# jepsen-io/comdb2

Hardware: AMD Instinct MI355X
Metric: serializable conflict checks/sec at 1–8 GPUs, % HBM roofline, vs host CPU (higher is better)
Workload: dtype u64

## Files before the change

### comdb2_amd/csrc/hsc_narrow.hip

```cpp
#include "hsc_device.h"
#include "hsc_internal.h"
#include "hsc_reldiff.h"

#include <hip/hip_runtime.h>

#include <algorithm>
#include <type_traits>

namespace hsc {

constexpr uint64_t kKeyPad = ~0ull;

__device__ __forceinline__ bool cnarrow_bound(const NarrowView &nv, uint64_t xg, const uint64_t *xw,
                                              size_t xs, bool upper, uint64_t &code)
{
    uint64_t acc = 0;
    int pos = 0, np = -1, xb = 0;
    for (int l = 0; l <= nv.W; ++l) {
        const uint64_t *cm = nv.cmeta + 8 * l;
        const uint64_t m = cm[0], pt = cm[1];
        uint64_t x = l ? xw[(size_t)(l - 1) * xs] : xg;
        if (np < 0) {
            const uint64_t d = (x ^ pt) & ~m;
            if (d) {
// ... 1240 lines not shown
        if (first[mid] < x)
            lo = mid + 1;
        else
            hi = mid;
    }
    put(lo);
}

static_assert(kTradMaxTiles <= 0xFFFF, "the packed table holds tile counts as u16");

hipError_t narrow_trad_build(const uint64_t *first, uint32_t ntiles, uint32_t m, uint32_t *trad,
                             uint16_t *trad16, hipStream_t s, int logmode)
{
    if (logmode && m < 64) return hipErrorInvalidValue;
    if (ntiles > kTradMaxTiles) return hipErrorInvalidValue;
    k_trad<<<(m + 8 + 255) / 256, 256, 0, s>>>(first, ntiles, m, logmode, trad, trad16);
    return hipGetLastError();
}

struct LocLds {
    uint32_t first, cdir, hist, trad, sbuf, rbuf, bytes;
};
__host__ __device__ inline LocLds loc_lds(const NarrowTiles &nt, uint32_t ntiles)
{
    LocLds L{};
    uint32_t o = 0;
    L.first = o;
    o += 8 * (nt.trad ? ((ntiles + 1) & ~1u) : dir16_lds_entries(nt.tdir));
    L.cdir = o;
    o += nt.rank_lsn32 ? 0 : 8 * dir16_lds_entries(nt.cdir);
    L.hist = o;
    o += 4 * ((ntiles + 3) & ~3u);
    o = (o + 15) & ~15u;
    L.trad = o;
    o += nt.trad ? (uint32_t)narrow_trad16_bytes(nt.trad_m) : 0;
    L.sbuf = o;
    o += nt.rank_lsn32 ? 0 : 8 * kLocTThreads;
    L.rbuf = o;
    o += 4 * (nt.rank_lsn32 ? kLocTThreads / 64 : kLocTThreads);
    L.bytes = o;
    return L;
}

template <int K, int kMode = -1>
__device__ __forceinline__ void trad_count(const uint64_t *first, const uint16_t *T, uint32_t m,
                                           int shift, uint32_t ntiles, const uint64_t (&x)[K],
                                           const bool (&act)[K], uint32_t (&out)[K])
{
    uint32_t l[K], h[K];
    const bool lg = kMode < 0 ? (shift & kTradLog) != 0 : kMode == 1;
    const int sv = shift & 0xFFFF;
#pragma unroll
    for (int k = 0; k < K; ++k) {
        const uint64_t b = lg ? trad_log_bucket(x[k], sv) : x[k] >> sv;
        const bool in = b < m;
        const uint32_t bi = in ? (uint32_t)b : 0;
        l[k] = in ? T[bi] : ntiles;
        h[k] = in ? T[bi + 1] : ntiles;
    }
    for (;;) {
        bool more = false;
#pragma unroll
        for (int k = 0; k < K; ++k) {
            if (l[k] < h[k]) {
                const uint32_t mid = (l[k] + h[k]) >> 1;
                const bool below = first[mid] < x[k];
                l[k] = below ? mid + 1 : l[k];
                h[k] = below ? h[k] : mid;
                more = true;
            }
        }
        if (!more) break;
    }
#pragma unroll
    for (int k = 0; k < K; ++k) out[k] = act[k] ? l[k] : 0;
}

template <int K>
struct LocDefer {
    uint32_t x[K], y[K], q[K];
    uint64_t snap[K];
};

__device__ __forceinline__ void zero_verdicts(const ProbeWork &work, uint32_t g)
{
    uint8_t *v = work.vout;
    const size_t nb = work.n_txn;
    const size_t head = std::min<size_t>(nb, (16 - ((uintptr_t)v & 15)) & 15);
    const size_t pieces = (nb - head) / 16, tail = head + 16 * pieces;
    const size_t t = (size_t)g * kLocTThreads + threadIdx.x, stride = (size_t)work.G * kLocTThreads;
    for (size_t i = t; i < pieces; i += stride) ((u32x4 *)(v + head))[i] = u32x4{0, 0, 0, 0};
    if (t < head) v[t] = 0;
    if (t < nb - tail) v[tail + t] = 0;
    if (work.bitmap)
        for (size_t i = t; i < ((size_t)work.n_txn + 63) / 64; i += stride) work.bitmap[i] = 0;
}

constexpr int kLocGeneral = 0, kLocFastLin = 1, kLocFastLog = 2;
template <int W, bool kTrad, int kShape = kLocGeneral>
__global__ __launch_bounds__(kLocTThreads) void k_locate_t(NarrowView nv, WinView wt, ProbeView p,
                                                           ProbeWork work, NarrowTiles nt,
                                                           uint8_t *verdict)
{
    constexpr bool kFast = kShape != kLocGeneral;
    static_assert(!kFast || (kTrad && (W == 1 || W == 2)), "fast shapes: bucket table, 1 or 2 words");
    constexpr int WR = 2 > W ? 2 : W;
    constexpr int K = 1, S = kLocTP;
    extern __shared__ __attribute__((aligned(16))) uint64_t lds64[];
    const uint32_t ntiles = wt.ntiles;
    const LocLds L = loc_lds(nt, ntiles);
    char *lb = (char *)lds64;
    uint64_t *tfirst = (uint64_t *)(lb + L.first);
    uint64_t *cdir = (uint64_t *)(lb + L.cdir);
    uint32_t *hist = (uint32_t *)(lb + L.hist);
    uint16_t *T = (uint16_t *)(lb + L.trad);
    const int lane = threadIdx.x & 63;
    uint64_t *sb = (uint64_t *)(lb + L.sbuf) + (threadIdx.x & ~63u);
    uint32_t *rb = (uint32_t *)(lb + L.rbuf) + (threadIdx.x & ~63u);
    const uint32_t g = xcd_chunk(blockIdx.x, (work.G + 7) / 8);
    if (g >= work.G) return;
    HSC_STAMP(work, 0, 0);
    if (g == 0 && threadIdx.x < 3) work.item_off[threadIdx.x] = 0;
    const uint32_t c0 = g * work.chunk;
    const uint32_t c1 = min(p.n, c0 + work.chunk);
    uint32_t qq[2][K], gg[2][K], tx[2][K];
    bool valid[2][K];
    uint64_t snap[2][K], xl[2][K][WR], xh[2][K][WR];
    uint4 R0[S][K], R1[S][K];
    uint32_t RT[S][K];
    uint64_t SS[S][K];
    auto load = [&](int s, int buf) {
#pragma unroll
        for (int k = 0; k < K; ++k) {
            const int j = s * K + k;
            qq[buf][k] = c0 + threadIdx.x + kLocTThreads * j;
            valid[buf][k] = qq[buf][k] < c1;
            const uint32_t q = valid[buf][k] ? qq[buf][k] : 0;
            const bool some = kFast || p.n;
            gg[buf][k] = some ? __builtin_nontemporal_load(p.gid + q) : 0;
            snap[buf][k] = some ? __builtin_nontemporal_load(p.snap + q) : 0;
            tx[buf][k] = some ? __builtin_nontemporal_load(p.txn + q) : 0;
#pragma unroll
            for (int w = 0; w < W; ++w) {
                xl[buf][k][w] = some ? __builtin_nontemporal_load(p.lo + (size_t)w * p.n + q) : 0;
                xh[buf][k][w] = some ? __builtin_nontemporal_load(p.hi + (size_t)w * p.n + q) : 0;
            }
        }
    };
    load(0, 0);
    const int tshift = nt.trad_shift;
    u64x2 sf[kTradFirstSlots], st[kTradSlots];
    uint64_t sft = 0;
    u64x2 sd[kDirSlots], sc[kDirSlots];
    if constexpr (kTrad) {
        const u64x2 *src = (const u64x2 *)wt.sp_w;
        const u64x2 *src16 = (const u64x2 *)nt.trad16;
#pragma unroll
        for (int j = 0; j < kTradFirstSlots; ++j) {
            const uint32_t i = threadIdx.x + kLocTThreads * j;
            sf[j] = *(i < ntiles / 2 ? src + i : src16);
        }
        sft = wt.sp_w[ntiles - 1];
#pragma unroll
        for (int j = 0; j < kTradSlots; ++j) {
            const uint32_t i = threadIdx.x + kLocTThreads * j;
            st[j] = src16[i < narrow_trad16_bytes(nt.trad_m) / 16 ? i : 0];
        }
    } else {
        dir16_stage_issue<kLocTThreads>(nt.tdir, sd);
    }
    const bool lsn32 = kFast || nt.rank_lsn32;
    if (!lsn32) dir16_stage_issue<kLocTThreads>(nt.cdir, sc);
    for (uint32_t i = threadIdx.x; i < ntiles; i += kLocTThreads) hist[i] = 0;
    if constexpr (kTrad) {
#pragma unroll
        for (int j = 0; j < kTradFirstSlots; ++j) {
            const uint32_t i = threadIdx.x + kLocTThreads * j;
            if (i < ntiles / 2) ((u64x2 *)tfirst)[i] = sf[j];
        }
        if ((ntiles & 1) && threadIdx.x == 0) tfirst[ntiles - 1] = sft;
#pragma unroll
        for (int j = 0; j < kTradSlots; ++j) {
            const uint32_t i = threadIdx.x + kLocTThreads * j;
            if (i < narrow_trad16_bytes(nt.trad_m) / 16) ((u64x2 *)T)[i] = st[j];
        }
    } else {
        dir16_stage_store<kLocTThreads>(nt.tdir, sd, tfirst);
    }
    if (!lsn32) dir16_stage_store<kLocTThreads>(nt.cdir, sc, cdir);
    __syncthreads();
    HSC_STAMP(work, 0, 1);
    const uint64_t *first = kTrad ? tfirst : wt.sp_w;
    uint64_t fbase[kFast ? W + 1 : 1] = {};
    const int ftz = nv.tz;
    if constexpr (kFast) {
#pragma unroll
        for (int i = 0; i <= W; ++i) fbase[i] = nv.base[i];
    }
    LocDefer<K> dfr;
#pragma unroll
    for (int k = 0; k < K; ++k) dfr.x[k] = 1, dfr.y[k] = 0;
    uint32_t sm[K][4];
    auto commit = [&](int s) {
#pragma unroll
        for (int k = 0; k < K; ++k) {
            uint4 &a = R0[s][k], &b = R1[s][k];
            bool drop_a = false, drop_b = false;
            if constexpr (kFast) {
                const uint32_t qr = a.w >> nt.qshift;
                drop_a = max(sm[k][0], sm[k][1]) < qr;
                drop_b = max(sm[k][2], sm[k][3]) < (b.w >> nt.qshift);
            }
            if (a.x != kNoTile32) {
                if (!drop_a)
                    a.x |= atomicAdd(&hist[a.x >> 12], 0x10001u) & 0xFFFFu;
                else
                    atomicAdd(&hist[a.x >> 12], 0x10000u), a.x = kNoTile32;
            }
            if (b.x != kNoTile32) {
                if (!drop_b)
                    b.x |= atomicAdd(&hist[b.x >> 12], 0x10001u) & 0xFFFFu;
                else
                    atomicAdd(&hist[b.x >> 12], 0x10000u), b.x = kNoTile32;
            }
        }
    };
#pragma unroll
    for (int s = 0; s < S; ++s) {
        const int cb = s & 1;
        uint64_t pm[K], psn[K];
        if (s > 0) {
#pragma unroll
            for (int k = 0; k < K; ++k) {
                pm[k] = dfr.x[k] <= dfr.y[k] ? tiles_max(wt, dfr.x[k], dfr.y[k]) : 0;
                psn[k] = dfr.snap[k];
            }
        }
        if (s + 1 < S) load(s + 1, cb ^ 1);
        uint64_t lo[K], hi[K];
#pragma unroll
        for (int k = 0; k < K; ++k) {
            if constexpr (kFast)
                locate_codes_fast<W>(ftz, fbase, valid[cb][k], gg[cb][k], xl[cb][k], xh[cb][k],
                                     lo[k], hi[k]);
            else
                locate_codes<W>(nv, p, valid[cb][k] ? qq[cb][k] : 0, gg[cb][k], xl[cb][k],
                                xh[cb][k], lo[k], hi[k]);
        }
        uint32_t rs[K];
        if (lsn32) {
#pragma unroll
            for (int k = 0; k < K; ++k) rs[k] = lsn32_rank(snap[cb][k], nt.rank_base);
        } else {
#pragma unroll
            for (int k = 0; k < K; ++k) rs[k] = 0, SS[s][k] = snap[cb][k];
        }
        uint32_t cnt[2 * K];
        {
            uint64_t keys[2 * K];
            bool act[2 * K];
#pragma unroll
            for (int k = 0; k < K; ++k) {
                keys[2 * k] = lo[k];
                keys[2 * k + 1] = dir_le(hi[k]);
                act[2 * k] = act[2 * k + 1] = valid[cb][k] && lo[k] <= hi[k];
            }
            if constexpr (kTrad)
                trad_count<2 * K, kFast ? kShape == kLocFastLog : -1>(tfirst, T, nt.trad_m, tshift,
                                                                      ntiles, keys, act, cnt);
            else
                dir16_count<2 * K>(nt.tdir, tfirst, keys, act, cnt);
        }
        if constexpr (kFast)
            if (s > 0) commit(s - 1);
#pragma unroll
        for (int k = 0; k < K; ++k) {
            dfr.x[k] = 1, dfr.y[k] = 0;
            R0[s][k].x = R1[s][k].x = kNoTile32;
            RT[s][k] = tx[cb][k];
            if constexpr (kFast) sm[k][0] = sm[k][1] = sm[k][2] = sm[k][3] = 0xFFFFFFFFu;
            if (!valid[cb][k]) continue;
            const uint32_t q = qq[cb][k];
            const uint32_t ca = cnt[2 * k], cbt = cnt[2 * k + 1];
            const uint32_t a = ca ? ca - 1 : 0;
            const uint32_t bt = cbt ? cbt - 1 : 0;
            uint4 r0 = make_uint4(kNoTile32, 0, 0, 0), r1 = r0;
            if (cbt > 0 && a <= bt && lo[k] <= hi[k]) {
                const uint64_t fa = first[a], fb = first[bt];
                const uint64_t lo_a = lo[k] <= fa ? 0 : lo[k] - fa;
                const uint64_t hi_a = a == bt ? (hi[k] < fa ? ~0ull : hi[k] - fa) : 0xFFFFFFFFull;
                const uint64_t hi_b = hi[k] < fb ? ~0ull : hi[k] - fb;
                const bool full_a = lo_a == 0 && (a < bt || hi_a >= 0xFFFFFFFFull);
                const bool use_a = lo_a <= 0xFFFFFFFFull && hi_a != ~0ull && lo_a <= hi_a;
                const bool use_b = a < bt && hi_b != ~0ull;
                const bool full_b = hi_b >= 0xFFFFFFFFull;
                dfr.x[k] = use_a && full_a ? a : a + 1;
                dfr.y[k] = a == bt ? (use_a && full_a ? a : 0) : (use_b && full_b ? bt : bt - 1);
                if (a == bt && !(use_a && full_a)) dfr.x[k] = 1, dfr.y[k] = 0;
                dfr.q[k] = q;
                dfr.snap[k] = snap[cb][k];
                const bool rec_a = use_a && !full_a, rec_b = use_b && !full_b;
                const uint32_t la = (uint32_t)lo_a, ha = (uint32_t)min(hi_a, 0xFFFFFFFFull);
                const uint32_t hb = (uint32_t)hi_b;
                if constexpr (kFast) {
                    if (rec_a) r0 = make_uint4(a << 12, la, ha, rs[k]);
                    if (rec_b) r1 = make_uint4(bt << 12, 0, hb, rs[k]);
                } else {
                    if (rec_a) r0 = make_uint4(a << 12 | atomicAdd(&hist[a], 1u), la, ha, rs[k]);
                    if (rec_b) r1 = make_uint4(bt << 12 | atomicAdd(&hist[bt], 1u), 0, hb, rs[k]);
                }
                if constexpr (kFast) {
                    const uint16_t *sa = nt.slots + (size_t)a * kSlots, *sb2 = nt.slots + (size_t)bt * kSlots;
                    const int sha = narrow_slot_shift(slot_span(tfirst, a, ntiles));
                    const int shb = narrow_slot_shift(slot_span(tfirst, bt, ntiles));
                    const uint32_t a0 = min(la >> sha, kSlots - 1), a1 = min(ha >> sha, kSlots - 1);
                    const uint32_t b1 = min(hb >> shb, kSlots - 1);
                    const bool try_a = rec_a && a1 - a0 <= 1, try_b = rec_b && b1 <= 1;
                    sm[k][0] = try_a ? sa[a0] : 0xFFFFFFFFu, sm[k][1] = try_a ? sa[a1] : 0xFFFFFFFFu;
                    sm[k][2] = try_b ? sb2[0] : 0xFFFFFFFFu, sm[k][3] = try_b ? sb2[b1] : 0xFFFFFFFFu;
                }
            }
            R0[s][k] = r0;
            R1[s][k] = r1;
        }
        if (s > 0) {
#pragma unroll
            for (int k = 0; k < K; ++k)
                if (pm[k] > psn[k]) verdict[RT[s - 1][k]] = 1;
        }
    }
    uint64_t dmax[K];
#pragma unroll
    for (int k = 0; k < K; ++k) dmax[k] = dfr.x[k] <= dfr.y[k] ? tiles_max(wt, dfr.x[k], dfr.y[k]) : 0;
    if constexpr (kFast) commit(S - 1);
    {
        if (!lsn32) {
            const uint64_t le_mask = lane == 63 ? ~0ull : ((2ull << lane) - 1);
            bool head[S][K];
            uint32_t slot[S][K];
            uint32_t H = 0;
#pragma unroll
            for (int s = 0; s < S; ++s)
#pragma unroll
                for (int k = 0; k < K; ++k) {
                    const uint64_t prev = __shfl_up(SS[s][k], 1, 64);
                    head[s][k] = lane == 0 || prev != SS[s][k];
                    const uint64_t m = __ballot(head[s][k]);
                    slot[s][k] = H + __popcll(m & le_mask) - 1;
                    H += __popcll(m);
                }
            for (uint32_t b0 = 0; b0 < H; b0 += 64) {
#pragma unroll
                for (int s = 0; s < S; ++s)
#pragma unroll
                    for (int k = 0; k < K; ++k)
                        if (head[s][k] && slot[s][k] - b0 < 64) sb[slot[s][k] - b0] = SS[s][k];
                __builtin_amdgcn_fence(__ATOMIC_RELEASE, "wavefront");
                __builtin_amdgcn_wave_barrier();
                __builtin_amdgcn_fence(__ATOMIC_ACQUIRE, "wavefront");
                const bool act[1] = {lane < H - b0};
                const uint64_t xs[1] = {act[0] ? dir_le(sb[lane]) : 0};
                uint32_t r[1];
                dir16_count<1>(nt.cdir, cdir, xs, act, r);
                rb[lane] = r[0];
                __builtin_amdgcn_fence(__ATOMIC_RELEASE, "wavefront");
                __builtin_amdgcn_wave_barrier();
                __builtin_amdgcn_fence(__ATOMIC_ACQUIRE, "wavefront");
#pragma unroll
                for (int s = 0; s < S; ++s)
#pragma unroll
                    for (int k = 0; k < K; ++k)
                        if (slot[s][k] - b0 < 64) R0[s][k].w = R1[s][k].w = rb[slot[s][k] - b0];
                __builtin_amdgcn_fence(__ATOMIC_RELEASE, "wavefront");
                __builtin_amdgcn_wave_barrier();
                __builtin_amdgcn_fence(__ATOMIC_ACQUIRE, "wavefront");
            }
        }
    }
    HSC_STAMP(work, 0, 2);
    for (uint32_t q = g * kLocTThreads + threadIdx.x; q < p.n_lock; q += work.G * kLocTThreads) {
        const uint32_t t = p.lock_table[q];
        if (t < wt.ntables && wt.table_max[t] > p.lock_snap[q]) verdict[p.lock_txn[q]] = 1;
    }
    __syncthreads();
    HSC_STAMP(work, 0, 3);
    {
        const uint32_t per = (ntiles + kLocTThreads - 1) / kLocTThreads;
        const uint32_t i0 = min(ntiles, threadIdx.x * per), i1 = min(ntiles, i0 + per);
        uint32_t sum = 0;
        constexpr uint32_t kCount = kFast ? 0xFFFFu : 0xFFFFFFFFu;
        for (uint32_t i = i0; i < i1; ++i) sum += hist[i] & kCount;
        uint32_t x = sum;
#pragma unroll
        for (int o = 1; o < 64; o <<= 1) {
            const uint32_t y = __shfl_up(x, o, 64);
            if (lane >= o) x += y;
        }
        uint32_t *wtot = (uint32_t *)(lb + L.rbuf);
        if (lane == 63) wtot[threadIdx.x >> 6] = x;
        __syncthreads();
        uint32_t run = x - sum;
        for (uint32_t w = 0; w < (threadIdx.x >> 6); ++w) run += wtot[w];
        const size_t ro = (size_t)g * ((ntiles + 3) & ~3u);
        for (uint32_t i = i0; i < i1; ++i) {
            const uint32_t h = hist[i], c = h & kCount;
            if constexpr (kFast)
                work.cmx[ro + i] = make_uint2(run << 16 | c, h >> 16);
            else
                work.cm[ro + i] = run << 16 | c;
            hist[i] = run;
            run += c;
        }
        __syncthreads();
        HSC_STAMP(work, 0, 4);
        uint4 *area = nt.recs + (size_t)g * 2 * work.chunk;
#pragma unroll
        for (int s = 0; s < S; ++s)
#pragma unroll
            for (int k = 0; k < K; ++k) {
                const uint4 a = R0[s][k], b = R1[s][k];
                if (a.x != kNoTile32)
                    area[hist[a.x >> 12] + (a.x & 0xFFFu)] = make_uint4(a.y, a.z, a.w, RT[s][k]);
                if (b.x != kNoTile32)
                    area[hist[b.x >> 12] + (b.x & 0xFFFu)] = make_uint4(b.y, b.z, b.w, RT[s][k]);
            }
        if (work.vout) zero_verdicts(work, g);
#pragma unroll
        for (int k = 0; k < K; ++k)
            if (dfr.x[k] <= dfr.y[k] && dmax[k] > dfr.snap[k]) verdict[RT[S - 1][k]] = 1;
    }
    HSC_STAMP(work, 0, 5);
}

bool narrow_locate_fast(const NarrowView &nv, const NarrowTiles &nt, const ProbeView &p)
{
    const int w = nv.W == 1 || nv.W == 2 ? nv.W : 0;
    const bool tr = nt.trad != nullptr;
    const bool log = tr && (nt.trad_shift & (int)kTradLog) != 0;
    return tr && w != 0 && !nv.comp && nv.lw == nv.W && nt.rank_lsn32 && p.n > 0 && !(log && w == 1);
}

hipError_t launch_locate_t(const NarrowView &nv, const WinView &wt, const ProbeView &p,
                           const ProbeWork &work, const NarrowTiles &nt, uint8_t *verdict,
                           hipStream_t s, int *shape)
{
    if (shape) *shape = -1;
    if (p.n == 0 && p.n_lock == 0) return hipSuccess;
    const size_t lds = loc_lds(nt, wt.ntiles).bytes;
    const bool tr = nt.trad != nullptr;
    if (tr ? wt.ntiles > kTradMaxTiles || nt.trad_m > kTradMax || !nt.trad16
           : nt.tdir.lds_n > (uint32_t)kDirLds)
        return hipErrorInvalidValue;
    if (!nt.rank_lsn32 && nt.cdir.lds_n > (uint32_t)kDirLds) return hipErrorInvalidValue;
    const int w = nv.W == 1 || nv.W == 2 ? nv.W : 0;
    const bool log = tr && (nt.trad_shift & (int)kTradLog) != 0;
    const bool fast = narrow_locate_fast(nv, nt, p);
    if (fast ? !work.cmx || work.cm : !work.cm || work.cmx) return hipErrorInvalidValue;
    if (shape) *shape = fast ? 1 : 0;
#define HSC_LOCATE(W_, TR_, ...)                                                                  \
    k_locate_t<W_, TR_, ##__VA_ARGS__><<<8 * ((work.G + 7) / 8), kLocTThreads, lds, s>>>(nv, wt, p, work, \
                                                                                   nt, verdict)
    if (fast && w == 1)
        HSC_LOCATE(1, true, kLocFastLin);
    else if (fast && !log)
        HSC_LOCATE(2, true, kLocFastLin);
    else if (fast)
        HSC_LOCATE(2, true, kLocFastLog);
    else if (w == 1 && tr)
        HSC_LOCATE(1, true);
    else if (w == 1)
        HSC_LOCATE(1, false);
    else if (w == 2 && tr)
        HSC_LOCATE(2, true);
    else if (w == 2)
        HSC_LOCATE(2, false);
    else if (tr)
        HSC_LOCATE(0, true);
    else
        HSC_LOCATE(0, false);
#undef HSC_LOCATE
    return hipGetLastError();
}

uint32_t narrow_tiles_chunk() { return kLocTP * kLocTThreads; }
uint32_t narrow_tiles_dir_lds() { return kDirLds; }

__device__ __forceinline__ void mark_hot(const ProbeWork &work)
{
    if (work.hot) __hip_atomic_store(work.hot, work.batch, __ATOMIC_RELAXED, __HIP_MEMORY_SCOPE_SYSTEM);
}

constexpr int kPlanSThreads = 512;
template <bool kWide>
__global__ __launch_bounds__(kPlanSThreads) void k_plan_s(ProbeWork work, uint32_t ntiles,
                                                          uint32_t *ctl, uint8_t *flags,
                                                          uint32_t n_txn, uint8_t *verdict)
{
    constexpr int TB = kPlanSThreads / 64;
    static_assert(TB % 4 == 0, "16-byte row pieces");
    constexpr uint32_t SR = kMaxChunks + 4;
    __shared__ __attribute__((aligned(16))) uint32_t sh[TB][SR];
    __shared__ uint16_t shl[kWide ? TB : 1][kWide ? SR : 1];
    const int lane = threadIdx.x & 63, w = threadIdx.x >> 6;
    const uint32_t t0 = blockIdx.x * TB, t = t0 + w;
    const uint32_t G = work.G, hs = hist_stride(G), rs = (ntiles + 3) & ~3u;
    for (uint32_t i = threadIdx.x; i < G * (TB / 4); i += kPlanSThreads) {
        const uint32_t g = i / (TB / 4), pc = i % (TB / 4);
        const uint32_t c = t0 + 4 * pc;
        if constexpr (kWide) {
            const u32x4 *src = (const u32x4 *)(work.cmx + (size_t)g * rs + c);
            const u32x4 z = {0, 0, 0, 0};
            const u32x4 a = c < rs ? src[0] : z, b = c < rs ? src[1] : z;
            sh[4 * pc][g] = a.x, sh[4 * pc + 1][g] = a.z, sh[4 * pc + 2][g] = b.x, sh[4 * pc + 3][g] = b.z;
            shl[4 * pc][g] = (uint16_t)a.y, shl[4 * pc + 1][g] = (uint16_t)a.w;
// ... 629 lines not shown
```

### comdb2_amd/csrc/hsc_probe_host.cpp

```cpp
#include "hsc_ctx.h"

#include <algorithm>
#include <cstdio>
#include <cstdlib>
#include <vector>

namespace {

struct PhaseMarker {
    hsc_ctx *c;
    const bool on;
    int next = 0;
    explicit PhaseMarker(hsc_ctx *c) : c(c), on(c->timing) {}
    int mark(int k)
    {
        if (!on) return HSC_OK;
        for (; next <= k; ++next) {
            if (!c->ev[next]) HIPCHK(c, hipEventCreate(&c->ev[next]));
            HIPCHK(c, hipEventRecord(c->ev[next], c->stream));
        }
        return HSC_OK;
    }
};

// ... 160 lines not shown
                 PhaseMarker &t)
{
    hipStream_t s = c->stream;
    c->probe_ntiles = wn.ntiles;
    c->probe_buckets = true;
    ProbeWork work{};
    if (!c->d_fulljoins.p) {
        HIPCHK(c, c->d_fulljoins.ensure(8));
        HIPCHK(c, hipMemset(c->d_fulljoins.p, 0, 8));
    }
    work.full_joins = c->d_fulljoins.as<uint32_t>();
    work.wave_fallbacks = work.full_joins + 1;
    work.chunk = narrow_tiles_chunk();
    uint32_t max_items;
    uint8_t *flags;
    HIPCHK_RC(c, bucket_scratch(c, b, p, wn.ntiles, 16, 8, work, max_items, flags));
    work.cursor = c->w_cursor.as<uint32_t>();
    work.item_tile = c->w_item_tile.as<uint32_t>();
    NarrowTiles ntl{};
    ntl.key32 = c->d_key32.as<uint32_t>();
    ntl.rank32 = c->d_rank32.as<uint32_t>();
    ntl.rank_lsn32 = c->rank_lsn32;
    ntl.rank_base = c->rank_base;
    ntl.cdir = c->cdir;
    ntl.tdir = c->tdir;
    ntl.trad = c->trad_m ? c->d_trad.as<uint32_t>() : nullptr;
    ntl.trad_m = c->trad_m;
    ntl.trad16 = c->trad_m ? c->d_trad16.as<uint16_t>() : nullptr;
    ntl.trad_shift = c->trad_shift;
    ntl.recs = c->w_trecs.as<uint4>();
    narrow_recent_view(ntl, c->d_recent.as<uint32_t>(), wn.ntiles, c->slot_qshift);
    const bool joins = p.n && wn.ntiles;
    const bool delta = pack_after_delta(c);
    bool column = false;
    if (joins) {
        if (!c->h_hot.p) {
            if (c->h_hot.ensure(16, true, true)) return ctx_fail(c, HSC_ENOMEM, "hot word");
            c->h_hot.as<volatile uint64_t>()[0] = 0;
            c->h_hot.as<volatile uint64_t>()[1] = 0;
        }
        work.hot = (uint64_t *)c->h_hot.dp;
        work.wide = work.hot + 1;
        work.batch = ++c->nt_batch;
        const uint64_t hot = *c->h_hot.as<volatile uint64_t>();
        column = !c->trad_log && !(hot && work.batch - hot <= hsc_ctx::kHotBatches);
        (column ? c->nt_column : c->nt_plan)++;
    }
    if (column) {
        work.vout = b->verdict;
        work.n_txn = (uint32_t)b->n_txn;
        work.bitmap = delta ? nullptr : b->bitmap;
    }
    HIPCHK_RC(c, t.mark(0));
    if (narrow_locate_fast(c->nv, ntl, p))
        work.cmx = c->w_tcode.as<uint2>();
    else
        work.cm = c->w_tcode.as<uint32_t>();
    int shape = -1;
    HIPCHK(c, launch_locate_t(c->nv, wn, p, work, ntl, flags, s, &shape));
    if (shape >= 0) (shape ? c->nt_fast : c->nt_general)++;
    HIPCHK_RC(c, t.mark(1));
    if (column) {
        HIPCHK_RC(c, t.mark(3));
        const uint64_t wide = c->h_hot.as<volatile uint64_t>()[1];
        const bool wave = work.cmx && !(wide && work.batch - wide <= hsc_ctx::kHotBatches);
        (wave ? c->nt_wave : c->nt_block)++;
        if (wave)
            HIPCHK(c, launch_join_wave(work, ntl, wn.n, wn.ntiles, flags, s));
        else
            HIPCHK(c, launch_join_col(work, ntl, wn.n, wn.ntiles, flags, s));
        HIPCHK_RC(c, tail_verdict(c, t, b, delta));
    } else if (joins) {
        work.bitmap = delta ? nullptr : b->bitmap;
        HIPCHK(c, launch_plan_s(work, wn.ntiles, c->w_items.as<uint32_t>(), s, flags,
                                (uint32_t)b->n_txn, b->verdict));
        HIPCHK_RC(c, t.mark(3));
        const uint32_t extra = c->trad_log ? 2048u : 512u;
        HIPCHK(c, launch_join_t(work, ntl, wn.n, wn.ntiles, max_items, b->verdict, s, extra));
        HIPCHK_RC(c, tail_verdict(c, t, b, delta));
    } else {
        HIPCHK_RC(c, tail_flags(c, t, b, flags));
    }
#ifdef HSC_STAMPS
    HIPCHK_RC(c, stamp_report(c, work, max_items, 6, 4));
#endif
    return HSC_OK;
}

int probe_ctiles(hsc_ctx *c, const hsc_probe_batch *b, const WinView &w, const ProbeView &p,
                 PhaseMarker &t)
{
    hipStream_t s = c->stream;
    CTiles ct = c->ctv;
    c->probe_ntiles = ct.ntiles;
    c->probe_buckets = true;
    ProbeWork work{};
    const size_t n1 = std::max<uint32_t>(p.n, 1);
    HIPCHK(c, c->p_code_lo.ensure(8 * (size_t)c->ct.WC * n1));
    HIPCHK(c, c->p_code_hi.ensure(8 * (size_t)c->ct.WC * n1));
    work.chunk = ctiles_chunk();
    uint32_t max_items;
    uint8_t *flags;
    HIPCHK_RC(c, bucket_scratch(c, b, p, ct.ntiles, 64, 4, work, max_items, flags));
    work.cm = c->w_tcode.as<uint32_t>();
    ct.recs = c->w_trecs.as<uint32_t>();
    ct.np = p.n;
    const WinView wt = with_tables(c->wc, w);
    HIPCHK_RC(c, t.mark(0));
    PointHash ph{};
    if (c->cph_nb) {
        ph.e = c->d_cph.as<uint64_t>();
        ph.nb = c->cph_nb;
        ph.WG = ct.WG;
        ph.gb = ct.gb;
        ph.rank_base = ct.rank_base;
        ph.flags = flags;
        ph.ep = c->cph_ep;
    }
    if (p.n)
        HIPCHK(c, compact_probes(p, c->ct, c->p_code_lo.as<uint64_t>(), c->p_code_hi.as<uint64_t>(), s, &ph));
    HIPCHK(c, launch_locate_c(ct, wt, p, c->p_code_lo.as<uint64_t>(), c->p_code_hi.as<uint64_t>(),
                              work, flags, s));
    HIPCHK_RC(c, t.mark(1));
    if (p.n && ct.ntiles) {
        const bool delta = pack_after_delta(c);
        work.bitmap = delta ? nullptr : b->bitmap;
        HIPCHK(c, launch_plan_s(work, ct.ntiles, c->w_items.as<uint32_t>(), s, flags,
                                (uint32_t)b->n_txn, b->verdict));
        HIPCHK_RC(c, t.mark(3));
        HIPCHK(c, launch_join_c(ct, work, max_items, b->verdict, s));
        HIPCHK_RC(c, tail_verdict(c, t, b, delta));
    } else {
        HIPCHK_RC(c, tail_flags(c, t, b, flags));
    }
#ifdef HSC_STAMPS
    HIPCHK_RC(c, stamp_report(c, work, max_items, 2, 7));
#endif
    return HSC_OK;
}

int probe_tiles(hsc_ctx *c, const hsc_probe_batch *b, const WinView &w, const ProbeView &p,
                PhaseMarker &t)
{
    hipStream_t s = c->stream;
    c->probe_ntiles = w.ntiles;
    c->probe_buckets = false;
    const uint32_t nt = std::max<uint32_t>(w.ntiles, 1);
    ProbeWork work{};
    work.lds_mode = w.ntiles <= (uint32_t)kHistCap;
    const size_t nwork = std::max<size_t>(p.n, p.n_lock);
    work.G = (uint32_t)std::min<size_t>(kMaxChunks, std::max<size_t>(1, (nwork + 2047) / 2048));
    work.chunk = (uint32_t)((p.n + work.G - 1) / work.G);
    HIPCHK(c, c->w_code.ensure(8 * (size_t)std::max<uint32_t>(p.n, 1)));
    HIPCHK(c, c->w_hist.ensure(4 * (size_t)work.G * nt));
    HIPCHK(c, c->w_counts.ensure(4 * ((size_t)nt + 1)));
    HIPCHK(c, c->w_bucket.ensure(4 * ((size_t)nt + 1)));
    HIPCHK(c, c->w_cursor.ensure(4 * ((size_t)nt + 1)));
    HIPCHK(c, c->w_items.ensure(4 * ((size_t)nt + 1)));
    HIPCHK(c, c->w_recs.ensure(8 * (size_t)rec_words(w.W) * 2 * std::max<uint32_t>(p.n, 1)));
    const uint32_t max_items = nt + (uint32_t)((2 * (size_t)p.n + kJoinChunk - 1) / kJoinChunk);
    HIPCHK(c, c->w_item_tile.ensure(4 * (size_t)max_items + 16));
    HIPCHK(c, c->w_item_desc.ensure(16 * (size_t)max_items + 16));
    work.item_desc = c->w_item_desc.as<uint4>();
    work.code = c->w_code.as<uint64_t>();
    work.hist = c->w_hist.as<uint32_t>();
    work.counts = c->w_counts.as<uint32_t>();
    work.bucket_off = c->w_bucket.as<uint32_t>();
// ... 126 lines not shown
```

Measured before the change: 3.746 billion.

## Split fast locate path: single-tile probes skip hi search, defer rare multi-tile probes

The fast locate kernel now counts only the lo key per probe and checks whether hi falls in the same tile. If it does, the second directory search and the second record are skipped. Probes that span several tiles are marked rare and deferred to a single batched flush per wave, or handled inline when the wave holds too many of them. The aim is to halve the directory searches in the common case and keep divergent multi-tile work out of the main loop. The cost is more complex control flow, wave ballots, and a change to which rank is written into the b records. The shared probe logic is moved into a helper, and the stamp indices shift by one.

```diff
diff --git a/comdb2_amd/csrc/hsc_narrow.hip b/comdb2_amd/csrc/hsc_narrow.hip
--- a/comdb2_amd/csrc/hsc_narrow.hip
+++ b/comdb2_amd/csrc/hsc_narrow.hip
@@ -1346,6 +1346,53 @@
     uint64_t snap[K];
 };
 
+template <bool kFast>
+__device__ __forceinline__ void locate_probe(const uint64_t *first, const uint64_t *tfirst,
+                                             uint32_t ntiles, const NarrowTiles &nt, uint32_t *hist,
+                                             uint64_t lo, uint64_t hi, uint32_t ca, uint32_t cbt,
+                                             uint32_t rs, uint64_t snap, uint4 &r0, uint4 &r1,
+                                             uint32_t &dx, uint32_t &dy, uint64_t &dsnap,
+                                             uint32_t (&sm)[4])
+{
+    const uint32_t a = ca ? ca - 1 : 0;
+    const uint32_t bt = cbt ? cbt - 1 : 0;
+    if (!(cbt > 0 && a <= bt && lo <= hi)) return;
+    const uint64_t fa = first[a], fb = first[bt];
+    const uint64_t lo_a = lo <= fa ? 0 : lo - fa;
+    const uint64_t hi_a = a == bt ? (hi < fa ? ~0ull : hi - fa) : 0xFFFFFFFFull;
+    const uint64_t hi_b = hi < fb ? ~0ull : hi - fb;
+    const bool full_a = lo_a == 0 && (a < bt || hi_a >= 0xFFFFFFFFull);
+    const bool use_a = lo_a <= 0xFFFFFFFFull && hi_a != ~0ull && lo_a <= hi_a;
+    const bool use_b = a < bt && hi_b != ~0ull;
+    const bool full_b = hi_b >= 0xFFFFFFFFull;
+    dx = use_a && full_a ? a : a + 1;
+    dy = a == bt ? (use_a && full_a ? a : 0) : (use_b && full_b ? bt : bt - 1);
+    if (a == bt && !(use_a && full_a)) dx = 1, dy = 0;
+    if constexpr (!kFast) dsnap = snap;
+    const bool rec_a = use_a && !full_a, rec_b = use_b && !full_b;
+    const uint32_t la = (uint32_t)lo_a, ha = (uint32_t)min(hi_a, 0xFFFFFFFFull);
+    const uint32_t hb = (uint32_t)hi_b;
+    if constexpr (kFast) {
+        if (rec_a) r0 = make_uint4(a << 12, la, ha, rs);
+        if (rec_b) r1 = make_uint4(bt << 12, 0, hb, rs);
+    } else {
+        if (rec_a) r0 = make_uint4(a << 12 | atomicAdd(&hist[a], 1u), la, ha, rs);
+        if (rec_b) r1 = make_uint4(bt << 12 | atomicAdd(&hist[bt], 1u), 0, hb, rs);
+    }
+    if constexpr (kFast) {
+        const uint16_t *sa = nt.slots + (size_t)a * kSlots, *sb2 = nt.slots + (size_t)bt * kSlots;
+        const int sha = narrow_slot_shift(slot_span(tfirst, a, ntiles));
+        const int shb = narrow_slot_shift(slot_span(tfirst, bt, ntiles));
+        const uint32_t a0 = min(la >> sha, kSlots - 1), a1 = min(ha >> sha, kSlots - 1);
+        const uint32_t b1 = min(hb >> shb, kSlots - 1);
+        const bool try_a = rec_a && a1 - a0 <= 1, try_b = rec_b && b1 <= 1;
+        sm[0] = try_a ? sa[a0] : 0xFFFFFFFFu, sm[1] = try_a ? sa[a1] : 0xFFFFFFFFu;
+        sm[2] = try_b ? sb2[0] : 0xFFFFFFFFu, sm[3] = try_b ? sb2[b1] : 0xFFFFFFFFu;
+    }
+}
+
+constexpr int kLocRareMax = 8;
+
 __device__ __forceinline__ void zero_verdicts(const ProbeWork &work, uint32_t g)
 {
     uint8_t *v = work.vout;
@@ -1464,139 +1511,170 @@
     LocDefer<K> dfr;
 #pragma unroll
     for (int k = 0; k < K; ++k) dfr.x[k] = 1, dfr.y[k] = 0;
-    uint32_t sm[K][4];
-    auto commit = [&](int s) {
-#pragma unroll
-        for (int k = 0; k < K; ++k) {
-            uint4 &a = R0[s][k], &b = R1[s][k];
-            bool drop_a = false, drop_b = false;
-            if constexpr (kFast) {
-                const uint32_t qr = a.w >> nt.qshift;
-                drop_a = max(sm[k][0], sm[k][1]) < qr;
-                drop_b = max(sm[k][2], sm[k][3]) < (b.w >> nt.qshift);
-            }
-            if (a.x != kNoTile32) {
-                if (!drop_a)
-                    a.x |= atomicAdd(&hist[a.x >> 12], 0x10001u) & 0xFFFFu;
+    uint64_t dmax[K] = {};
+    if constexpr (kFast) {
+        static_assert(K == 1, "one probe per sub-chunk and thread");
+        constexpr int kMode = kShape == kLocFastLog;
+        constexpr uint32_t kFree = 0xFFFFFFFFu;
+        uint64_t phi = 0;
+        uint32_t pend = kFree;
+        auto commit = [&](bool has, uint32_t &x, uint32_t rs, uint32_t m0, uint32_t m1) {
+            if (!has) return;
+            if (!(max(m0, m1) < rs >> nt.qshift))
+                x |= atomicAdd(&hist[x >> 12], 0x10001u) & 0xFFFFu;
+            else
+                atomicAdd(&hist[x >> 12], 0x10000u), x = kNoTile32;
+        };
+        auto full = [&](bool act, uint64_t lo, uint64_t hi, uint32_t ca, uint32_t rs, uint32_t txn,
+                        uint4 &o0, uint4 &o1) {
+            const uint64_t keys[1] = {dir_le(hi)};
+            const bool on[1] = {act};
+            uint32_t cbt[1];
+            trad_count<1, kMode>(tfirst, T, nt.trad_m, tshift, ntiles, keys, on, cbt);
+            uint4 r0 = make_uint4(kNoTile32, 0, 0, 0), r1 = r0;
+            uint32_t dx = 1, dy = 0, sm[4] = {0xFFFFFFFFu, 0xFFFFFFFFu, 0xFFFFFFFFu, 0xFFFFFFFFu};
+            uint64_t none = 0;
+            if (act)
+                locate_probe<true>(tfirst, tfirst, ntiles, nt, hist, lo, hi, ca, cbt[0], rs, 0, r0, r1, dx,
+                                   dy, none, sm);
+            const uint64_t mx = dx <= dy ? tiles_max(wt, dx, dy) : 0;
+            commit(r0.x != kNoTile32, r0.x, rs, sm[0], sm[1]);
+            commit(r1.x != kNoTile32, r1.x, rs, sm[2], sm[3]);
+            if (dx <= dy && mx - nt.rank_base + 1 > rs) verdict[txn] = 1;
+            if (act) o0 = make_uint4(r0.x, r0.y, r0.z, rs), o1 = r1;
+        };
+        auto flush = [&]() {
+            const bool on = pend != kFree;
+            const int sub = on ? (int)(pend & 3) : S;
+            uint32_t l0 = 0, l1 = 0, rs = 0, txn = 0;
+#pragma unroll
+            for (int s = 0; s < S; ++s) {
+                l0 = sub == s ? R0[s][0].y : l0, l1 = sub == s ? R0[s][0].z : l1;
+                rs = sub == s ? R0[s][0].w : rs, txn = sub == s ? RT[s][0] : txn;
+            }
+            uint4 o0 = make_uint4(kNoTile32, 0, 0, 0), o1 = o0;
+            full(on, (uint64_t)l1 << 32 | l0, phi, pend >> 2, rs, txn, o0, o1);
+#pragma unroll
+            for (int s = 0; s < S; ++s)
+                if (sub == s) R0[s][0] = o0, R1[s][0] = o1;
+            pend = kFree;
+        };
+        uint32_t sm0 = 0xFFFFFFFFu, sm1 = 0xFFFFFFFFu;
+        bool cand = false;
+#pragma unroll
+        for (int s = 0; s < S; ++s) {
+            const int cb = s & 1;
+            if (s + 1 < S) load(s + 1, cb ^ 1);
+            uint64_t lo, hi;
+            locate_codes_fast<W>(ftz, fbase, valid[cb][0], gg[cb][0], xl[cb][0], xh[cb][0], lo, hi);
+            const uint32_t rs = lsn32_rank(snap[cb][0], nt.rank_base);
+            const bool act = valid[cb][0] && lo <= hi;
+            uint32_t cnt[1];
+            {
+                const uint64_t keys[1] = {lo};
+                const bool on[1] = {act};
+                trad_count<1, kMode>(tfirst, T, nt.trad_m, tshift, ntiles, keys, on, cnt);
+            }
+            const uint32_t ca = cnt[0];
+            if (s > 0) commit(cand, R0[s - 1][0].x, R0[s - 1][0].w, sm0, sm1);
+            const uint32_t a = ca ? ca - 1 : 0;
+            const bool lastt = ca == ntiles;
+            const bool one = act && ca > 0 && (lastt || hi < tfirst[lastt ? a : ca]);
+            const bool rare = act && !one;
+            const uint64_t fa = tfirst[a];
+            const uint64_t lo_a = lo - fa, hi_a = hi - fa;
+            cand = one && lo_a <= 0xFFFFFFFFull;
+            const uint32_t la = (uint32_t)lo_a, ha = (uint32_t)min(hi_a, 0xFFFFFFFFull);
+            R0[s][0] = make_uint4(cand ? a << 12 : kNoTile32, la, ha, rs);
+            R1[s][0] = make_uint4(kNoTile32, 0, 0, 0);
+            RT[s][0] = tx[cb][0];
+            {
+                const uint16_t *sa = nt.slots + (size_t)a * kSlots;
+                const int sha = narrow_slot_shift(slot_span(tfirst, a, ntiles));
+                const uint32_t a0 = min(la >> sha, kSlots - 1), a1 = min(ha >> sha, kSlots - 1);
+                const bool try_a = cand && a1 - a0 <= 1;
+                sm0 = try_a ? sa[a0] : 0xFFFFFFFFu, sm1 = try_a ? sa[a1] : 0xFFFFFFFFu;
+            }
+            const uint64_t rm = __ballot(rare);
+            if (rm == 0) continue;
+            if (__popcll(rm) > kLocRareMax || __ballot(rare && pend != kFree)) {
+                full(rare, lo, hi, ca, rs, tx[cb][0], R0[s][0], R1[s][0]);
+                continue;
+            }
+            if (rare) {
+                R0[s][0].y = (uint32_t)lo, R0[s][0].z = (uint32_t)(lo >> 32);
+                phi = hi, pend = ca << 2 | s;
+            }
+        }
+        HSC_STAMP(work, 0, 2);
+        if (__ballot(pend != kFree)) flush();
+        commit(cand, R0[S - 1][0].x, R0[S - 1][0].w, sm0, sm1);
+    } else {
+#pragma unroll
+        for (int s = 0; s < S; ++s) {
+            const int cb = s & 1;
+            uint64_t pm[K], psn[K];
+            if (s > 0) {
+#pragma unroll
+                for (int k = 0; k < K; ++k) {
+                    pm[k] = dfr.x[k] <= dfr.y[k] ? tiles_max(wt, dfr.x[k], dfr.y[k]) : 0;
+                    psn[k] = dfr.snap[k];
+                }
+            }
+            if (s + 1 < S) load(s + 1, cb ^ 1);
+            uint64_t lo[K], hi[K];
+#pragma unroll
+            for (int k = 0; k < K; ++k)
+                locate_codes<W>(nv, p, valid[cb][k] ? qq[cb][k] : 0, gg[cb][k], xl[cb][k], xh[cb][k],
+                                lo[k], hi[k]);
+            uint32_t rs[K];
+            if (lsn32) {
+#pragma unroll
+                for (int k = 0; k < K; ++k) rs[k] = lsn32_rank(snap[cb][k], nt.rank_base);
+            } else {
+#pragma unroll
+                for (int k = 0; k < K; ++k) rs[k] = 0, SS[s][k] = snap[cb][k];
+            }
+            uint32_t cnt[2 * K];
+            {
+                uint64_t keys[2 * K];
+                bool act[2 * K];
+#pragma unroll
+                for (int k = 0; k < K; ++k) {
+                    keys[2 * k] = lo[k];
+                    keys[2 * k + 1] = dir_le(hi[k]);
+                    act[2 * k] = act[2 * k + 1] = valid[cb][k] && lo[k] <= hi[k];
+                }
+                if constexpr (kTrad)
+                    trad_count<2 * K>(tfirst, T, nt.trad_m, tshift, ntiles, keys, act, cnt);
                 else
-                    atomicAdd(&hist[a.x >> 12], 0x10000u), a.x = kNoTile32;
-            }
-            if (b.x != kNoTile32) {
-                if (!drop_b)
-                    b.x |= atomicAdd(&hist[b.x >> 12], 0x10001u) & 0xFFFFu;
-                else
-                    atomicAdd(&hist[b.x >> 12], 0x10000u), b.x = kNoTile32;
-            }
-        }
-    };
-#pragma unroll
-    for (int s = 0; s < S; ++s) {
-        const int cb = s & 1;
-        uint64_t pm[K], psn[K];
-        if (s > 0) {
+                    dir16_count<2 * K>(nt.tdir, tfirst, keys, act, cnt);
+            }
 #pragma unroll
             for (int k = 0; k < K; ++k) {
-                pm[k] = dfr.x[k] <= dfr.y[k] ? tiles_max(wt, dfr.x[k], dfr.y[k]) : 0;
-                psn[k] = dfr.snap[k];
-            }
-        }
-        if (s + 1 < S) load(s + 1, cb ^ 1);
-        uint64_t lo[K], hi[K];
-#pragma unroll
-        for (int k = 0; k < K; ++k) {
-            if constexpr (kFast)
-                locate_codes_fast<W>(ftz, fbase, valid[cb][k], gg[cb][k], xl[cb][k], xh[cb][k],
-                                     lo[k], hi[k]);
-            else
-                locate_codes<W>(nv, p, valid[cb][k] ? qq[cb][k] : 0, gg[cb][k], xl[cb][k],
-                                xh[cb][k], lo[k], hi[k]);
-        }
-        uint32_t rs[K];
-        if (lsn32) {
-#pragma unroll
-            for (int k = 0; k < K; ++k) rs[k] = lsn32_rank(snap[cb][k], nt.rank_base);
-        } else {
-#pragma unroll
-            for (int k = 0; k < K; ++k) rs[k] = 0, SS[s][k] = snap[cb][k];
-        }
-        uint32_t cnt[2 * K];
-        {
-            uint64_t keys[2 * K];
-            bool act[2 * K];
-#pragma unroll
-            for (int k = 0; k < K; ++k) {
-                keys[2 * k] = lo[k];
-                keys[2 * k + 1] = dir_le(hi[k]);
-                act[2 * k] = act[2 * k + 1] = valid[cb][k] && lo[k] <= hi[k];
-            }
-            if constexpr (kTrad)
-                trad_count<2 * K, kFast ? kShape == kLocFastLog : -1>(tfirst, T, nt.trad_m, tshift,
-                                                                      ntiles, keys, act, cnt);
-            else
-                dir16_count<2 * K>(nt.tdir, tfirst, keys, act, cnt);
-        }
-        if constexpr (kFast)
-            if (s > 0) commit(s - 1);
-#pragma unroll
-        for (int k = 0; k < K; ++k) {
-            dfr.x[k] = 1, dfr.y[k] = 0;
-            R0[s][k].x = R1[s][k].x = kNoTile32;
-            RT[s][k] = tx[cb][k];
-            if constexpr (kFast) sm[k][0] = sm[k][1] = sm[k][2] = sm[k][3] = 0xFFFFFFFFu;
-            if (!valid[cb][k]) continue;
-            const uint32_t q = qq[cb][k];
-            const uint32_t ca = cnt[2 * k], cbt = cnt[2 * k + 1];
-            const uint32_t a = ca ? ca - 1 : 0;
-            const uint32_t bt = cbt ? cbt - 1 : 0;
-            uint4 r0 = make_uint4(kNoTile32, 0, 0, 0), r1 = r0;
-            if (cbt > 0 && a <= bt && lo[k] <= hi[k]) {
-                const uint64_t fa = first[a], fb = first[bt];
-                const uint64_t lo_a = lo[k] <= fa ? 0 : lo[k] - fa;
-                const uint64_t hi_a = a == bt ? (hi[k] < fa ? ~0ull : hi[k] - fa) : 0xFFFFFFFFull;
-                const uint64_t hi_b = hi[k] < fb ? ~0ull : hi[k] - fb;
-                const bool full_a = lo_a == 0 && (a < bt || hi_a >= 0xFFFFFFFFull);
-                const bool use_a = lo_a <= 0xFFFFFFFFull && hi_a != ~0ull && lo_a <= hi_a;
-                const bool use_b = a < bt && hi_b != ~0ull;
-                const bool full_b = hi_b >= 0xFFFFFFFFull;
-                dfr.x[k] = use_a && full_a ? a : a + 1;
-                dfr.y[k] = a == bt ? (use_a && full_a ? a : 0) : (use_b && full_b ? bt : bt - 1);
-                if (a == bt && !(use_a && full_a)) dfr.x[k] = 1, dfr.y[k] = 0;
-                dfr.q[k] = q;
-                dfr.snap[k] = snap[cb][k];
-                const bool rec_a = use_a && !full_a, rec_b = use_b && !full_b;
-                const uint32_t la = (uint32_t)lo_a, ha = (uint32_t)min(hi_a, 0xFFFFFFFFull);
-                const uint32_t hb = (uint32_t)hi_b;
-                if constexpr (kFast) {
-                    if (rec_a) r0 = make_uint4(a << 12, la, ha, rs[k]);
-                    if (rec_b) r1 = make_uint4(bt << 12, 0, hb, rs[k]);
-                } else {
-                    if (rec_a) r0 = make_uint4(a << 12 | atomicAdd(&hist[a], 1u), la, ha, rs[k]);
-                    if (rec_b) r1 = make_uint4(bt << 12 | atomicAdd(&hist[bt], 1u), 0, hb, rs[k]);
-                }
-                if constexpr (kFast) {
-                    const uint16_t *sa = nt.slots + (size_t)a * kSlots, *sb2 = nt.slots + (size_t)bt * kSlots;
-                    const int sha = narrow_slot_shift(slot_span(tfirst, a, ntiles));
-                    const int shb = narrow_slot_shift(slot_span(tfirst, bt, ntiles));
-                    const uint32_t a0 = min(la >> sha, kSlots - 1), a1 = min(ha >> sha, kSlots - 1);
-                    const uint32_t b1 = min(hb >> shb, kSlots - 1);
-                    const bool try_a = rec_a && a1 - a0 <= 1, try_b = rec_b && b1 <= 1;
-                    sm[k][0] = try_a ? sa[a0] : 0xFFFFFFFFu, sm[k][1] = try_a ? sa[a1] : 0xFFFFFFFFu;
-                    sm[k][2] = try_b ? sb2[0] : 0xFFFFFFFFu, sm[k][3] = try_b ? sb2[b1] : 0xFFFFFFFFu;
-                }
-            }
-            R0[s][k] = r0;
-            R1[s][k] = r1;
-        }
-        if (s > 0) {
-#pragma unroll
-            for (int k = 0; k < K; ++k)
-                if (pm[k] > psn[k]) verdict[RT[s - 1][k]] = 1;
-        }
-    }
-    uint64_t dmax[K];
-#pragma unroll
-    for (int k = 0; k < K; ++k) dmax[k] = dfr.x[k] <= dfr.y[k] ? tiles_max(wt, dfr.x[k], dfr.y[k]) : 0;
-    if constexpr (kFast) commit(S - 1);
+                dfr.x[k] = 1, dfr.y[k] = 0;
+                R0[s][k].x = R1[s][k].x = kNoTile32;
+                RT[s][k] = tx[cb][k];
+                if (!valid[cb][k]) continue;
+                uint4 r0 = make_uint4(kNoTile32, 0, 0, 0), r1 = r0;
+                uint32_t none[4];
+                locate_probe<false>(first, tfirst, ntiles, nt, hist, lo[k], hi[k], cnt[2 * k],
+                                    cnt[2 * k + 1], rs[k], snap[cb][k], r0, r1, dfr.x[k], dfr.y[k],
+                                    dfr.snap[k], none);
+                R0[s][k] = r0;
+                R1[s][k] = r1;
+            }
+            if (s > 0) {
+#pragma unroll
+                for (int k = 0; k < K; ++k)
+                    if (pm[k] > psn[k]) verdict[RT[s - 1][k]] = 1;
+            }
+        }
+        HSC_STAMP(work, 0, 2);
+#pragma unroll
+        for (int k = 0; k < K; ++k)
+            dmax[k] = dfr.x[k] <= dfr.y[k] ? tiles_max(wt, dfr.x[k], dfr.y[k]) : 0;
+    }
     {
         if (!lsn32) {
             const uint64_t le_mask = lane == 63 ? ~0ull : ((2ull << lane) - 1);
@@ -1641,13 +1719,13 @@
             }
         }
     }
-    HSC_STAMP(work, 0, 2);
+    HSC_STAMP(work, 0, 3);
     for (uint32_t q = g * kLocTThreads + threadIdx.x; q < p.n_lock; q += work.G * kLocTThreads) {
         const uint32_t t = p.lock_table[q];
         if (t < wt.ntables && wt.table_max[t] > p.lock_snap[q]) verdict[p.lock_txn[q]] = 1;
     }
     __syncthreads();
-    HSC_STAMP(work, 0, 3);
+    HSC_STAMP(work, 0, 4);
     {
         const uint32_t per = (ntiles + kLocTThreads - 1) / kLocTThreads;
         const uint32_t i0 = min(ntiles, threadIdx.x * per), i1 = min(ntiles, i0 + per);
@@ -1676,7 +1754,7 @@
             run += c;
         }
         __syncthreads();
-        HSC_STAMP(work, 0, 4);
+        HSC_STAMP(work, 0, 5);
         uint4 *area = nt.recs + (size_t)g * 2 * work.chunk;
 #pragma unroll
         for (int s = 0; s < S; ++s)
@@ -1686,14 +1764,17 @@
                 if (a.x != kNoTile32)
                     area[hist[a.x >> 12] + (a.x & 0xFFFu)] = make_uint4(a.y, a.z, a.w, RT[s][k]);
                 if (b.x != kNoTile32)
-                    area[hist[b.x >> 12] + (b.x & 0xFFFu)] = make_uint4(b.y, b.z, b.w, RT[s][k]);
+                    area[hist[b.x >> 12] + (b.x & 0xFFFu)] =
+                        make_uint4(b.y, b.z, kFast ? a.w : b.w, RT[s][k]);
             }
         if (work.vout) zero_verdicts(work, g);
-#pragma unroll
-        for (int k = 0; k < K; ++k)
-            if (dfr.x[k] <= dfr.y[k] && dmax[k] > dfr.snap[k]) verdict[RT[S - 1][k]] = 1;
-    }
-    HSC_STAMP(work, 0, 5);
+        if constexpr (!kFast) {
+#pragma unroll
+            for (int k = 0; k < K; ++k)
+                if (dfr.x[k] <= dfr.y[k] && dmax[k] > dfr.snap[k]) verdict[RT[S - 1][k]] = 1;
+        }
+    }
+    HSC_STAMP(work, 0, 6);
 }
 
 bool narrow_locate_fast(const NarrowView &nv, const NarrowTiles &nt, const ProbeView &p)
diff --git a/comdb2_amd/csrc/hsc_probe_host.cpp b/comdb2_amd/csrc/hsc_probe_host.cpp
--- a/comdb2_amd/csrc/hsc_probe_host.cpp
+++ b/comdb2_amd/csrc/hsc_probe_host.cpp
@@ -266,7 +266,7 @@
         HIPCHK_RC(c, tail_flags(c, t, b, flags));
     }
 #ifdef HSC_STAMPS
-    HIPCHK_RC(c, stamp_report(c, work, max_items, 6, 4));
+    HIPCHK_RC(c, stamp_report(c, work, max_items, 7, 4));
 #endif
     return HSC_OK;
 }
```

Measured after the change: 3.620 billion. 0.966x the previous value.
